# DoumanAsh/compu

Hardware: AMD Instinct MI355X
Metric: decompressed GB/s (whole node), batched 64 KiB DEFLATE blocks; % HBM peak (higher is better)
Workload: dtype u8

## Files before the change

compu_amd/csrc/api.hip:

```cpp
#include <stdio.h>
#include <stdlib.h>
#include <string.h>

#include <mutex>
#include <new>
#include <thread>
#include <vector>

#include "chip_internal.h"
#include "lz4_enc_core.h"

using namespace chip;

namespace {

struct Hooks {
    chip_malloc_fn malloc_fn = nullptr;
    chip_free_fn free_fn = nullptr;
    void *opaque = nullptr;
    void *alloc(size_t n) const { return malloc_fn ? malloc_fn(opaque, n) : malloc(n); }
    void release(void *p) const
    {
        if (!p) return;
        if (free_fn) free_fn(opaque, p);
        else free(p);
    }
};
std::mutex g_hooks_mu;
Hooks g_hooks;
Hooks current_hooks()
{
    std::lock_guard<std::mutex> lk(g_hooks_mu);
    return g_hooks;
}

bool device_ok()
{
    int n = 0;
    return hipGetDeviceCount(&n) == hipSuccess && n > 0;
}

struct Meta {
    uint64_t in_off, out_off;
    uint32_t in_len, out_cap, out_len, in_used;
    int32_t status;
    uint32_t resume[RESUME_WORDS];
};

BatchArgs batch_args(int format, size_t n, const void *in_base, const uint64_t *in_off, const uint32_t *in_len, void *out_base,
                     const uint64_t *out_off, const uint32_t *out_cap, uint32_t *out_len, uint32_t *in_used, int32_t *status)
{
    BatchArgs a;
    a.in_base = (const uint8_t *)in_base;
    a.in_off = in_off;
    a.in_len = in_len;
    a.out_base = (uint8_t *)out_base;
    a.out_off = out_off;
    a.out_cap = out_cap;
    a.out_len = out_len;
    a.in_used = in_used;
    a.status = status;
    a.n = (uint32_t)n;
    a.format = format;
    a.stats = nullptr;
    a.resume = nullptr;
#ifdef CHIP_STATS
    a.stats = getenv("CHIP_STATS_PTR") ? (unsigned long long *)strtoull(getenv("CHIP_STATS_PTR"), nullptr, 0) : nullptr;
#endif
    return a;
}

void pipes_trim();

}

extern "C" {

int chip_device_count(void)
{
    int n = 0;
    if (hipGetDeviceCount(&n) != hipSuccess) return 0;
    return n;
}

int chip_set_device(int device) { return hipSetDevice(device) == hipSuccess ? CHIP_OK : CHIP_E_NO_DEVICE; }

const char *chip_version(void) { return "compu-hip 0.1 (gfx950)"; }

void chip_set_allocator(chip_malloc_fn malloc_fn, chip_free_fn free_fn, void *opaque)
{
    std::lock_guard<std::mutex> lk(g_hooks_mu);
    g_hooks.malloc_fn = (malloc_fn && free_fn) ? malloc_fn : nullptr;
    g_hooks.free_fn = (malloc_fn && free_fn) ? free_fn : nullptr;
    g_hooks.opaque = (malloc_fn && free_fn) ? opaque : nullptr;
}

void *chip_device_alloc(size_t size)
{
    void *p = nullptr;
    if (hipMalloc(&p, size ? size : 4) != hipSuccess) return nullptr;
    return p;
}
void chip_device_free(void *ptr)
{
    if (ptr) (void)hipFree(ptr);
}
void *chip_pinned_alloc(size_t size)
{
    void *p = nullptr;
    if (hipHostMalloc(&p, size ? size : 4, hipHostMallocDefault) != hipSuccess) return nullptr;
    return p;
}
void chip_pinned_free(void *ptr)
{
    if (ptr) (void)hipHostFree(ptr);
}
int chip_memcpy_h2d(void *dst, const void *src, size_t size, void *stream)
{
    return hipMemcpyAsync(dst, src, size, hipMemcpyHostToDevice, (hipStream_t)stream) == hipSuccess ? CHIP_OK : CHIP_E_LAUNCH;
}
int chip_memcpy_d2h(void *dst, const void *src, size_t size, void *stream)
{
    return hipMemcpyAsync(dst, src, size, hipMemcpyDeviceToHost, (hipStream_t)stream) == hipSuccess ? CHIP_OK : CHIP_E_LAUNCH;
}
int chip_stream_sync(void *stream) { return hipStreamSynchronize((hipStream_t)stream) == hipSuccess ? CHIP_OK : CHIP_E_LAUNCH; }
int chip_trim(void)
{
    pipes_trim();
    return chip::release_scratch() == hipSuccess ? CHIP_OK : CHIP_E_LAUNCH;
}


int chip_decode_batch(int format, size_t n, const void *in_base, const uint64_t *in_off, const uint32_t *in_len,
                      void *out_base, const uint64_t *out_off, const uint32_t *out_cap, uint32_t *out_len,
                      uint32_t *in_used, int32_t *status, void *stream)
{
    return chip_decode_batch_ex(format, 0, n, in_base, in_off, in_len, out_base, out_off, out_cap, out_len, in_used, status, stream);
}

static bool members_flag_ok(int format, uint32_t flags)
{
    if ((format == CHIP_FMT_LZ4_BLOCK || format == CHIP_FMT_LZ4) && flags) return false;
    if (!(flags & CHIP_F_MEMBERS)) return true;
    if (flags & CHIP_F_COMPU_STATUS) return false;
    return format == CHIP_FMT_GZIP || format == CHIP_FMT_AUTO || format == CHIP_FMT_ZSTD || format == CHIP_FMT_DETECT;
}

int chip_decode_batch_ex(int format, uint32_t flags, size_t n, const void *in_base, const uint64_t *in_off, const uint32_t *in_len,
                         void *out_base, const uint64_t *out_off, const uint32_t *out_cap, uint32_t *out_len,
                         uint32_t *in_used, int32_t *status, void *stream)
{
    if (flags & ~(uint32_t)(CHIP_F_COMPU_STATUS | CHIP_F_MEMBERS)) return CHIP_E_INVALID;
    if (!members_flag_ok(format, flags)) return CHIP_E_INVALID;
    if (n == 0) return CHIP_OK;
    if (n > 0x7fffffffull || !in_base || !in_off || !in_len || !out_base || !out_off || !out_cap || !out_len || !in_used ||
        !status || ((uintptr_t)in_base & 3u))
        return CHIP_E_INVALID;
    if (!device_ok()) return CHIP_E_NO_DEVICE;
    BatchArgs a = batch_args(format, n, in_base, in_off, in_len, out_base, out_off, out_cap, out_len, in_used, status);
    a.flags = flags;
    hipError_t e;
    switch (format) {
    case CHIP_FMT_DEFLATE:
    case CHIP_FMT_ZLIB:
    case CHIP_FMT_GZIP:
    case CHIP_FMT_AUTO: e = launch_inflate(a, nullptr, (hipStream_t)stream); break;
    case CHIP_FMT_ZSTD: e = launch_zstd(a, nullptr, 0, (hipStream_t)stream); break;
    case CHIP_FMT_BROTLI: e = launch_brotli_decode(a, (hipStream_t)stream); break;
    case CHIP_FMT_LZ4_BLOCK:
    case CHIP_FMT_LZ4: e = launch_lz4(a, nullptr, (hipStream_t)stream); break;
    case CHIP_FMT_DETECT:
        e = launch_routed(a, nullptr, (hipStream_t)stream);
        break;
    default: return CHIP_E_INVALID;
    }
    return e == hipSuccess ? CHIP_OK : CHIP_E_LAUNCH;
}

int chip_decode_batch_sizes(int format, uint32_t flags, size_t n, const void *in_base, const uint64_t *in_off, const uint32_t *in_len,
                            uint64_t *out_size, uint32_t *in_used, int32_t *status, void *stream)
{
    if (flags & ~(uint32_t)CHIP_F_MEMBERS) return CHIP_E_INVALID;
    if (!members_flag_ok(format, flags)) return CHIP_E_INVALID;
    switch (format) {
    case CHIP_FMT_DEFLATE:
    case CHIP_FMT_ZLIB:
    case CHIP_FMT_GZIP:
    case CHIP_FMT_AUTO:
    case CHIP_FMT_ZSTD:
    case CHIP_FMT_LZ4_BLOCK:
    case CHIP_FMT_LZ4:
    case CHIP_FMT_DETECT: break;
    default: return CHIP_E_INVALID;
    }
    if (n == 0) return CHIP_OK;
    if (n > 0x7fffffffull || !in_base || !in_off || !in_len || !out_size || !in_used || !status || ((uintptr_t)in_base & 3u))
        return CHIP_E_INVALID;
    if (!device_ok()) return CHIP_E_NO_DEVICE;
    BatchArgs a = batch_args(format, n, in_base, in_off, in_len, nullptr, nullptr, nullptr, nullptr, in_used, status);
    a.flags = flags;
    hipError_t e;
    if (format == CHIP_FMT_ZSTD) e = launch_zstd(a, out_size, 0, (hipStream_t)stream);
    else if (format == CHIP_FMT_LZ4_BLOCK || format == CHIP_FMT_LZ4) e = launch_lz4(a, out_size, (hipStream_t)stream);
    else if (format == CHIP_FMT_DETECT) e = launch_routed(a, out_size, (hipStream_t)stream);
    else e = launch_inflate(a, out_size, (hipStream_t)stream);
    return e == hipSuccess ? CHIP_OK : CHIP_E_LAUNCH;
}

}

namespace {

struct DeviceGuard {
    int prev = -1;
    bool ok = true;
    explicit DeviceGuard(int device)
    {
        if (hipGetDevice(&prev) != hipSuccess) prev = -1;
        if (device >= 0 && device != prev) ok = hipSetDevice(device) == hipSuccess;
    }
// ... 1228 lines not shown
```

compu_amd/csrc/chip_internal.h:

```cpp
#pragma once
#include <hip/hip_runtime.h>
#include <stddef.h>
#include <stdint.h>

#include "../../include/compu_hip.h"
#include "zstd_enc_core.h"

namespace chip {

constexpr int32_t ST_RUNNING = 0x7fffffff;

constexpr int32_t Z_NEED_DICT = 2;
constexpr int32_t Z_DATA_ERROR = -3;

constexpr int32_t ZSTD_E_GENERIC = 1;
constexpr int32_t ZSTD_E_PREFIX_UNKNOWN = 10;
constexpr int32_t ZSTD_E_FRAMEPARAM_UNSUPPORTED = 14;
constexpr int32_t ZSTD_E_WINDOW_TOO_LARGE = 16;
constexpr int32_t ZSTD_E_CORRUPTION = 20;
constexpr int32_t ZSTD_E_CHECKSUM_WRONG = 22;
constexpr int32_t ZSTD_E_DICT_WRONG = 32;

constexpr uint32_t RESUME_WORDS = 6;

constexpr uint32_t ZRES_HDR = 24;
constexpr uint32_t ZSAVE_WORDS = 2312;
constexpr size_t ZRES_BYTES = (size_t)(ZRES_HDR + ZSAVE_WORDS) * 4 + 64;

struct BatchArgs {
    const uint8_t *in_base;
    const uint64_t *in_off;
    const uint32_t *in_len;
    uint8_t *out_base;
    const uint64_t *out_off;
    const uint32_t *out_cap;
    uint32_t *out_len;
    uint32_t *in_used;
    int32_t *status;
    uint32_t n;
    int32_t format;
    unsigned long long *stats;
    uint32_t *resume;
    const uint32_t *sel = nullptr;
    const uint32_t *sel_n = nullptr;
    uint32_t flags = 0;
};
struct ZTokArgs {
    const chip_zstd_block *blocks;
    const uint32_t *seq_base;
    uint32_t *tok;
    uint32_t *res;
    uint64_t window;
};
constexpr uint32_t ZTOK_SLOT_SLACK = 8736;
hipError_t launch_zstd_tokens(const BatchArgs &a, const ZTokArgs &tk, hipStream_t stream);
hipError_t launch_zstd_xxh(const uint8_t *p, uint32_t n, uint32_t *got, hipStream_t stream);
hipError_t launch_zstd_xxh_update(const uint8_t *p, uint32_t n, const chip_xxh64_state &st, chip_xxh64_state *out, hipStream_t stream);
constexpr uint32_t F_COMPU_STATUS = 1u;
constexpr uint32_t F_MEMBERS = 2u;

hipError_t launch_inflate(const BatchArgs &a, uint64_t *out_size, hipStream_t stream);
hipError_t enqueue_inflate_sizes(const BatchArgs &a, uint64_t *out_size, uint32_t *scratch, uint32_t *counter, uint32_t blocks, hipStream_t stream);
hipError_t enqueue_inflate_members(const BatchArgs &a, uint64_t *out_size, uint32_t *scratch, uint32_t *counter, uint32_t blocks, hipStream_t stream);
hipError_t enqueue_inflate_markers(const BatchArgs &a, const uint32_t *bit0, uint32_t *scratch, uint32_t *counter, uint32_t blocks, hipStream_t stream);
hipError_t launch_zstd(const BatchArgs &a, uint64_t *out_size, int window_log_max, hipStream_t stream);
hipError_t enqueue_zstd_sizes(const BatchArgs &a, uint64_t *out_size, int wlog_max, hipStream_t stream);
hipError_t enqueue_zstd_members(const BatchArgs &a, int wlog_max, hipStream_t stream);
hipError_t enqueue_zstd_members_sizes(const BatchArgs &a, uint64_t *out_size, int wlog_max, hipStream_t stream);
hipError_t launch_lz4(const BatchArgs &a, uint64_t *out_size, hipStream_t stream);
hipError_t launch_lz4_xxh(const uint8_t *p, uint64_t n, uint32_t *got, hipStream_t stream);
bool lz4_encode_args_ok(int format, int level, int strategy);
hipError_t launch_lz4_encode(const BatchArgs &a, int level, int strategy, hipStream_t stream);
hipError_t release_scratch();
void release_scratch_of(hipStream_t stream);
hipError_t launch_route(const BatchArgs &a, uint64_t *out_size, uint32_t *sel_inflate, uint32_t *sel_zstd, uint32_t *counts, hipStream_t stream);
hipError_t launch_routed(const BatchArgs &a, uint64_t *out_size, hipStream_t stream);
hipError_t launch_detect(size_t n, const uint8_t *in_base, const uint64_t *in_off, const uint32_t *in_len, int32_t *kind,
                         hipStream_t stream);
hipError_t launch_deflate_l1(const BatchArgs &a, int level, uint32_t flags, uint32_t check_seed, uint64_t total_before,
                             uint32_t *check_out, hipStream_t stream);

constexpr uint32_t ZF_FIRST = 1u, ZF_LAST = 2u, ZF_ONESHOT = 4u;
struct ZEncStream {
    uint32_t rep[3], pad;
    zenc::Xxh xxh;
};
hipError_t launch_zstd_encode(const BatchArgs &a, int level, int strategy, uint32_t wlog_single, uint32_t wlog_window, uint32_t flags,
                              ZEncStream *stream_state, hipStream_t stream);

struct BEncStream {
    uint32_t ring[4];
};
hipError_t launch_brotli_encode(const BatchArgs &a, int quality, int lgwin, uint32_t flags, BEncStream *stream_state, hipStream_t stream);

constexpr uint32_t BRES_WORDS = 16;
static_assert(BRES_WORDS <= ZRES_HDR, "the brotli checkpoint fits the header the streaming code copies");
hipError_t launch_brotli_decode(const BatchArgs &a, hipStream_t stream);
size_t brotli_scratch_bytes_of(hipStream_t stream);

__device__ __forceinline__ int32_t detect_kind(const uint8_t *b, uint32_t len)
{
    if (len < 2) return CHIP_DETECT_NONE;
    const uint32_t b0 = b[0], b1 = b[1];
    if (b0 == 0x1f && b1 == 0x8b) return CHIP_DETECT_GZIP;
    if (((b0 << 8) | b1) % 31 == 0 && (b0 & 0x8f) == 0x08 && b0 != 0x68) {
        const uint32_t rows[8] = {0x1d5b99d7u, 0x195795d3u, 0x155391cfu, 0x114f8dcbu, 0x0d4b89c7u, 0x094785c3u, 0x054381deu, 0x015e9cdau};
        const uint32_t r = rows[b0 >> 4];
        if (b1 == (r >> 24) || b1 == ((r >> 16) & 0xff) || b1 == ((r >> 8) & 0xff) || b1 == (r & 0xff)) return CHIP_DETECT_ZLIB;
    }
    if (len < 4) return CHIP_DETECT_NONE;
    return (b0 == 0x28 && b1 == 0xb5 && b[2] == 0x2f && b[3] == 0xfd) ? CHIP_DETECT_ZSTD : CHIP_DETECT_UNKNOWN;
}

#define LDS_AS __attribute__((address_space(3)))
#define GAS __attribute__((address_space(1)))

__device__ __forceinline__ uint32_t lane_id() { return threadIdx.x & 63u; }
__device__ __forceinline__ uint64_t lanemask_lt() { return (1ull << lane_id()) - 1ull; }
__device__ __forceinline__ uint32_t rdlane(uint32_t v, uint32_t l)
{
    return (uint32_t)__builtin_amdgcn_readlane((int)v, (int)l);
}
__device__ __forceinline__ uint32_t rdfirst(uint32_t v) { return (uint32_t)__builtin_amdgcn_readfirstlane((int)v); }
template <typename T>
__device__ __forceinline__ T *rdfirst_ptr(T *p)
{
    const uint64_t v = (uint64_t)(uintptr_t)p;
    return (T *)(uintptr_t)(((uint64_t)rdfirst((uint32_t)(v >> 32)) << 32) | rdfirst((uint32_t)v));
}

template <int CTRL, int ROW_MASK = 0xf>
__device__ __forceinline__ uint32_t dpp_or_zero(uint32_t v)
{
    return (uint32_t)__builtin_amdgcn_update_dpp(0, (int)v, CTRL, ROW_MASK, 0xf, false);
}

__device__ __forceinline__ uint32_t wave_incl_scan(uint32_t v)
{
    v += dpp_or_zero<0x111>(v);
    v += dpp_or_zero<0x112>(v);
    v += dpp_or_zero<0x114>(v);
    v += dpp_or_zero<0x118>(v);
    v += dpp_or_zero<0x142, 0xa>(v);
    v += dpp_or_zero<0x143, 0xc>(v);
    return v;
}

__device__ __forceinline__ uint32_t wave_incl_max_scan(uint32_t v)
{
    uint32_t t;
    t = dpp_or_zero<0x111>(v); v = v > t ? v : t;
    t = dpp_or_zero<0x112>(v); v = v > t ? v : t;
    t = dpp_or_zero<0x114>(v); v = v > t ? v : t;
    t = dpp_or_zero<0x118>(v); v = v > t ? v : t;
    t = dpp_or_zero<0x142, 0xa>(v); v = v > t ? v : t;
    t = dpp_or_zero<0x143, 0xc>(v); v = v > t ? v : t;
    return v;
}

__device__ __forceinline__ uint32_t wave_shr1(uint32_t v) { return dpp_or_zero<0x138>(v); }

#define WSYNC() __syncthreads()
#define LSYNC() asm volatile("s_waitcnt lgkmcnt(0)" ::: "memory")

}
```

compu_amd/csrc/inflate_unit.h:

```cpp
#pragma once
#include "chip_internal.h"
#include "wave_checksums.h"

namespace chip {

typedef uint32_t u32x2 __attribute__((ext_vector_type(2)));
typedef uint32_t u32x4 __attribute__((ext_vector_type(4)));
typedef u32x4 u32x4_u __attribute__((aligned(1)));
typedef u32x4 u32x4_a4 __attribute__((aligned(4)));
template <typename T>
__device__ __forceinline__ GAS T *rdfirst_gptr(T *p)
{
    return (GAS T *)rdfirst_ptr(p);
}

#ifndef CHIP_PHASE_FN
#define CHIP_PHASE_FN __attribute__((always_inline))
#endif

#ifndef CHIP_INFLATE_SPEC
#define CHIP_INFLATE_SPEC 0
#endif
#ifndef CHIP_INFLATE_MARKERS
#define CHIP_INFLATE_MARKERS 0
#endif
#if CHIP_INFLATE_SPEC
#define SPEC_PARAM , uint32_t &sp_reach
#define SPEC_ARG , sp_reach
#else
#define SPEC_PARAM
#define SPEC_ARG
#endif

#ifdef CHIP_STATS
#define STAT_DECL unsigned long long st_[24] = {0}; unsigned long long st_t0_ = 0
#define STAT_T0() (st_t0_ = __builtin_readcyclecounter())
#define STAT_ACC(i) do { unsigned long long n_ = __builtin_readcyclecounter(); st_[i] += n_ - st_t0_; st_t0_ = n_; } while (0)
#define STAT_ADD(i, v) (st_[i] += (unsigned long long)(v))
#define STAT_PARAM , unsigned long long *st_, unsigned long long &st_t0_
#define STAT_ARG , st_, st_t0_
#else
#define STAT_DECL
#define STAT_T0()
#define STAT_ACC(i)
#define STAT_ADD(i, v)
#define STAT_PARAM
#define STAT_ARG
#endif

enum : uint32_t { K_LIT = 0, K_LEN = 1, K_EOB = 2, K_BAD = 3 };
__device__ __forceinline__ constexpr uint32_t mk_entry(uint32_t cl, uint32_t eb, uint32_t kind, uint32_t base)
{
    return cl | (eb << 4) | (kind << 8) | (base << 16);
}

constexpr int LIT_ROOT = 9;
constexpr int DIST_ROOT = 8;
constexpr int CL_ROOT = 7;

constexpr uint32_t F_HALT = 1u << 15, F_INV = 1u << 26, F_LEN = 1u << 31;
constexpr uint32_t D_BAD = 1u << 10, D_LONG = 1u << 15;
static_assert(15 - LIT_ROOT < 8 && 15 - DIST_ROOT < 8, "a root entry's index bit count leaves its bits [4:3] clear");
static_assert((2u << (15 - DIST_ROOT)) - 2u < 256u, "the distance sub-tables fit the 256 units that a root entry's offset spans");

__device__ __forceinline__ uint32_t make_final(uint32_t sym, uint32_t len)
{
    if (sym < 256) return len | (len << 10) | (sym << 16);
    if (sym == 256) return len | (len << 10) | F_HALT;
    if (sym >= 286) return len | (len << 10) | F_HALT | F_INV;
    const uint32_t s = sym - 257;
    uint32_t eb = 0, base = 3 + s;
    if (s == 28) base = 258;
    else if (s >= 8) {
        eb = (s >> 2) - 1;
        base = 3 + ((4 + (s & 3)) << eb);
    }
    return len | (eb << 5) | ((len + eb) << 10) | ((512u | base) << 16) | F_LEN;
}
__device__ __forceinline__ uint32_t make_dist16(uint32_t sym, uint32_t len)
{
    if (sym >= 30) return len | D_BAD;
    if (sym < 4) return len | (sym << 8);
    return len | (((sym >> 1) - 1) << 4) | ((2 + (sym & 1)) << 8);
}

#ifndef CHIP_S_BITS
#define CHIP_S_BITS 320
#define CHIP_XT_BITS 1536
#define CHIP_XT_BITS_FIXED 3072
#define CHIP_ROW_TOKENS 256
#endif
constexpr uint32_t S_BITS = CHIP_S_BITS;
constexpr uint32_t XT_BITS = CHIP_XT_BITS;
#ifndef CHIP_XT_BITS_FIXED
#define CHIP_XT_BITS_FIXED CHIP_XT_BITS
#endif
constexpr uint32_t XT_BITS_FIXED = CHIP_XT_BITS_FIXED;
constexpr uint32_t ROW_TOKENS = CHIP_ROW_TOKENS;
static_assert(S_BITS % 32 == 0 && ROW_TOKENS % 4 == 0 && 64 * ROW_TOKENS < 65536, "geometry");
constexpr uint32_t SEG_WORDS = S_BITS / 32 + 1;
constexpr uint32_t SEG_SHIFT = 24;
constexpr uint32_t SEG_MAGIC = ((1u << SEG_SHIFT) + S_BITS - 1) / S_BITS;
constexpr bool seg_magic_ok()
{
    for (uint32_t x = 0; x < 64u * S_BITS + 4096u; x++)
        if (((x * SEG_MAGIC) >> SEG_SHIFT) != x / S_BITS) return false;
    return true;
}
static_assert(seg_magic_ok() && (64u * S_BITS + 4096u) * (uint64_t)SEG_MAGIC < (1ull << 32), "segment index by multiplication");
constexpr uint32_t WIN_DW = (31 + 64 * S_BITS + 48 + 96 + 31) / 32 + 3;
constexpr uint32_t HDR_IN_DW = 192;

constexpr size_t ROWS_WORDS = (size_t)64 * ROW_TOKENS;
static_assert(64ull * ROW_TOKENS * 258 < (1ull << 32), "count_tokens() sums a super-round's output lengths in 32 bits");
__device__ __forceinline__ uint32_t row_base(uint32_t l) { return (l >> 3) * (8u * ROW_TOKENS) + (l & 7u) * 4u; }
__device__ __forceinline__ uint32_t row_word(uint32_t k) { return k + (k >> 2) * 28u; }

__device__ __forceinline__ uint32_t tok_olen(uint32_t t) { return (t & 512u) ? t & 0x1ffu : 1u + (t >> 31); }

struct HuffMeta {
    uint32_t limit15[16];
    uint32_t offs[16];
    uint32_t maxlen;
};

#ifndef CHIP_CHUNK_BYTES
#define CHIP_CHUNK_BYTES 2560
#endif
#ifndef CHIP_COPY_LANE_MAX
#define CHIP_COPY_LANE_MAX 32
#endif
constexpr uint32_t CHUNK_BYTES = CHIP_CHUNK_BYTES;
constexpr uint32_t COPY_LANE_MAX = CHIP_COPY_LANE_MAX;
constexpr uint32_t MQ_CAP = 128;
constexpr uint32_t IMG_WORDS = CHUNK_BYTES / 4 + 8;
constexpr uint32_t TOK_RING = 4;
static_assert(CHUNK_BYTES % 4 == 0 && CHUNK_BYTES >= 1024 && COPY_LANE_MAX % 16 == 0 && IMG_WORDS % 2 == 0, "geometry");

constexpr uint32_t FLUSH_BYTES = 4 * (IMG_WORDS + 2 * MQ_CAP + 64 * TOK_RING + 128 + 4);
constexpr uint32_t HDR_BYTES = 4 * HDR_IN_DW + 4 * (1 << CL_ROOT) + 80 + sizeof(HuffMeta) + 64 + 320 + 2 * 288 + 2 * 32 + 2 * sizeof(HuffMeta);
constexpr uint32_t PHASE_BYTES = 8 * WIN_DW > FLUSH_BYTES ? (8 * WIN_DW > HDR_BYTES ? 8 * WIN_DW : HDR_BYTES) : (FLUSH_BYTES > HDR_BYTES ? FLUSH_BYTES : HDR_BYTES);
#ifndef CHIP_LDS_BYTES
#define CHIP_LDS_BYTES 8960
#endif
constexpr uint32_t POOL_WORDS = (CHIP_LDS_BYTES - 2 * 512 - 2 * 256 - PHASE_BYTES) / 4;
constexpr uint32_t POOL_U16 = 2 * POOL_WORDS;
constexpr uint32_t DIST_SUB_BYTES = 2 * (POOL_U16 - 256);

struct alignas(16) WaveLds {
    union {
        struct {
            uint32_t win[WIN_DW];
            uint32_t bm[WIN_DW];
        } w;
        struct {
            uint32_t inbuf[HDR_IN_DW];
            uint32_t cl_lut[1 << CL_ROOT];
            uint32_t cl_sorted[20];
            HuffMeta cl_h;
            uint32_t count[16];
            uint8_t lens[320];
            uint16_t lit_sorted[288];
            uint16_t dist_sorted[32];
            HuffMeta lit_h, dist_h;
        } hdr;
        struct {
            uint32_t out[IMG_WORDS];
            uint2 mq[MQ_CAP];
            uint32_t tok[64 * TOK_RING];
            uint32_t pk[128];
            uint32_t trash[4];
        } fl;
        uint32_t phase_words_[PHASE_BYTES / 4];
    };
    uint16_t lit_root[1 << LIT_ROOT];
    uint16_t dist_root[1 << DIST_ROOT];
    uint32_t pool[POOL_WORDS];
};
static_assert(sizeof(WaveLds) <= CHIP_LDS_BYTES, "the waves per CU that CHIP_LDS_BYTES stands for");
static_assert(POOL_WORDS >= 413 + 142, "the tables of any valid block fit");
#ifndef CHIP_EXP_ALLOW_SMALL_LDS
static_assert(sizeof(WaveLds) >= 2048 * 4, "wave_crc32 needs 8 KB");
#endif

__device__ __forceinline__ uint32_t canon_index(const HuffMeta &H, uint32_t x15, uint32_t &l)
{
    l = 1;
    if (x15 >= H.limit15[15]) return 0xffffffffu;
#pragma unroll
    for (int j = 1; j < 15; j++) l += (x15 >= H.limit15[j]) ? 1u : 0u;
    return H.offs[l] + ((x15 - H.limit15[l - 1]) >> (15 - l));
}

struct CanonLim {
    uint32_t lim[16];
};
__device__ __forceinline__ CanonLim canon_limits(const HuffMeta &H)
{
    CanonLim c;
#pragma unroll
    for (int j = 0; j < 16; j++) c.lim[j] = rdfirst(H.limit15[j]);
    return c;
}
template <int LO, int HI>
__device__ __forceinline__ uint32_t canon_index_in(const HuffMeta &H, const CanonLim &c, uint32_t x15, uint32_t &l)
{
    l = LO;
#pragma unroll
    for (int j = LO; j < HI; j++) l += (x15 >= c.lim[j]) ? 1u : 0u;
    return H.offs[l] + ((x15 - H.limit15[l - 1]) >> (15 - l));
}

template <typename SortedT, typename MakeT>
__device__ __forceinline__ int canon_prep(uint32_t *count, const uint8_t *lens, int n_, bool code_lengths, SortedT *sorted, HuffMeta &H, MakeT make STAT_PARAM)
{
    const uint32_t lane = lane_id();
    const int n = (int)rdfirst((uint32_t)n_);
    if (lane < 16) count[lane] = 0;
    WSYNC();
    for (int s = lane; s < n; s += 64) {
        uint32_t l = lens[s];
        if (l) atomicAdd(&count[l], 1u);
    }
    WSYNC();
    const uint32_t c = lane >= 1 && lane <= 15 ? count[lane] : 0u;
    const uint32_t cincl = wave_incl_scan(c);
    const uint32_t off = cincl - c;
    const uint32_t lim = wave_incl_scan(lane <= 15 ? c << (15u - (lane & 15u)) : 0u);
    const uint32_t present = (uint32_t)__ballot(c != 0);
    const uint32_t maxlen = present ? 31u - (uint32_t)__clz((int)present) : 0u;
    const bool over = __any(lane <= 15 && lim > 32768u);
    const int left = rdlane(lim, 15) < 32768u ? 1 : 0;
    if (lane <= 15) {
        H.limit15[lane] = lim;
        H.offs[lane] = off;
        count[lane] = off;
    }
    if (lane == 0) H.maxlen = maxlen;
    WSYNC();
    if (maxlen == 0) return 1;
    if (over) return -1;
    if (left > 0 && (code_lengths || maxlen != 1)) return -1;
    for (int base = 0; base < n; base += 64) {
        STAT_ADD(19, 1);
        const int s = base + (int)lane;
        const uint32_t l = s < n ? lens[s] : 0;
        uint64_t same = ~0ull;
#pragma unroll
        for (uint32_t b = 0; b < 4; b++) {
            const bool bit = (l >> b) & 1u;
            const uint64_t m = __ballot(bit);
// ... 698 lines not shown
                nfirst = before < npieces ? nx : 0xffffffffu;
            }
            asm volatile("s_waitcnt vmcnt(0)" ::: "memory");
            slot_r = 0;
#pragma unroll
            for (uint32_t k = 0; k < TOK_RING; k++) fetch(k);
        }
        const uint32_t xcap = cap - (opos - mis);
        {
            const uint32_t xe = run < xcap ? run : xcap;
            for (uint32_t xq = 16u + 16u * lane; xq + 16u <= xe; xq += 1024u) *(GAS u32x4_a4 *)(base + xq) = *(const LDS_AS u32x4 *)(img + xq);
            const uint32_t xt = xe < 16u ? 16u : xe & ~15u;
            const uint32_t xb = lane < 16u ? lane : xt + (lane - 16u);
            if (lane < 32u && xb >= mis && xb < xe) ((GAS uint8_t *)base)[xb] = img[xb];
        }
        WSYNC();
        STAT_ACC(18);
        opos += run - mis;
        opos_ = opos;
        const bool no_room = opos > cap || (too_far && opos == cap);
        if (no_room || too_far) {
            if (no_room) {
                opos_ = cap;
                ovf[0] = cstart;
                ovf[1] = mis;
                ovf[2] = xcap;
            }
            status = no_room ? CHIP_NEED_OUTPUT : Z_DATA_ERROR;
            return false;
        }
        if (c0 >= ntok) return true;
    }
}
constexpr size_t SCRATCH_WORDS = ROWS_WORDS;


enum : uint32_t { R_JOIN = 1, R_LIMIT = 2, R_EOB = 3, R_NEED_INPUT = 4, R_BAD = 5 };

__device__ CHIP_PHASE_FN uint32_t walk_round(WaveLds &L, const InWin &w, const uint32_t B_, const uint32_t end_bit_, uint32_t *rows_, const uint32_t xt_bits,
                                             uint32_t &ntok_out, uint32_t &term_why, uint32_t &term_pos STAT_PARAM)
{
    const uint32_t lane = lane_id();
    const uint32_t B = rdfirst(B_), end_bit = rdfirst(end_bit_);
    GAS const uint32_t *const g32 = rdfirst_gptr(w.g32);
    const uint32_t total_dw = rdfirst(w.total_dw);
    GAS uint32_t *const myrow = rdfirst_gptr(rows_) + row_base(lane);
    const uint32_t D0 = B >> 5;
    WSYNC();
    {
        constexpr uint32_t WIN_Q = WIN_DW / 4, WIN_R = WIN_DW % 4;
        constexpr uint32_t BM_A = (WIN_DW + 3u) & ~3u;
        constexpr uint32_t BM_Q = (2u * WIN_DW - BM_A) / 4, BM_TAIL = (2u * WIN_DW - BM_A) % 4;
        constexpr uint32_t EDGE_LO = WIN_R + (BM_A - WIN_DW);
        constexpr uint32_t EDGE_LANES = 4u + EDGE_LO + BM_TAIL;
        constexpr uint32_t PER_LANE = (WIN_Q + 63) / 64;
        static_assert(offsetof(WaveLds, w.win) == 0 && offsetof(WaveLds, w.bm) == 4 * WIN_DW && BM_Q <= WIN_Q && EDGE_LANES <= 64, "window staging");
        uint32_t *const ww = L.w.win;
        const uint32_t rem = total_dw - D0;
        static_assert(PER_LANE <= 4, "the quads per lane below");
        auto quad = [&](uint32_t j) -> u32x4 {
            const uint32_t k = 64u * j + lane;
            if ((64u * j + 63u < WIN_Q || k < WIN_Q) && 4u * k + 4u <= rem) return *(GAS const u32x4_a4 *)(g32 + D0 + 4u * k);
            return u32x4{0, 0, 0, 0};
        };
        const u32x4 v0 = quad(0), v1 = quad(1), v2 = quad(2), v3 = quad(3);
        uint32_t ni = 4u * (rem >> 2) + lane;
        bool nput = ni < rem && ni < 4u * WIN_Q;
        if (lane >= 4u) {
            const uint32_t j = lane - 4u;
            ni = j < EDGE_LO ? 4u * WIN_Q + j : 2u * WIN_DW - BM_TAIL + (j - EDGE_LO);
            nput = j < EDGE_LO + BM_TAIL;
        }
        uint32_t nv = 0;
        if (nput && ni < rem && ni < WIN_DW) nv = g32[D0 + ni];
#pragma unroll
        for (uint32_t j = 0; j < PER_LANE; j++) {
            const uint32_t k = 64u * j + lane;
            if (64u * j + 63u < WIN_Q || k < WIN_Q) *(u32x4 *)(ww + 4u * k) = j == 0 ? v0 : j == 1 ? v1 : j == 2 ? v2 : v3;
            if (64u * j + 63u < BM_Q || k < BM_Q) *(u32x4 *)(ww + BM_A + 4u * k) = u32x4{0, 0, 0, 0};
        }
        if (nput) ww[ni] = nv;
    }
    LSYNC();
    STAT_ACC(1);
    STAT_ADD(8, 1);
    const uint32_t s0 = B + lane * S_BITS;
    const uint32_t own_end = s0 + S_BITS;
    uint32_t hard = own_end + xt_bits;
    {
        const uint32_t sr_end = B + 64u * S_BITS;
        hard = hard < sr_end ? hard : sr_end;
        hard = hard < end_bit ? hard : end_bit;
    }
    const uint32_t wbase = 32u * D0;
    const uint32_t own_end_r = own_end - wbase, hard_r = hard - wbase;
    uint32_t q = s0 - wbase, tl = 0, nst = 0;
    uint32_t jb = 0, z = 0;
    bool run = s0 < end_bit;
    uint32_t nx;
    {
        const uint32_t *wp = (const uint32_t *)((const uint8_t *)L.w.win + ((q >> 3) & ~3u));
        nx = __builtin_amdgcn_alignbit(wp[1], wp[0], q);
    }
    auto token = [&](uint32_t &tok) -> bool {
        const uint32_t p = q;
        const uint32_t a = (p >> 3) & ~3u;
        const uint32_t bit = 1u << (p & 31u);
        const uint32_t mine = p < own_end_r ? bit : 0u;
        const uint32_t old = atomicOr((uint32_t *)((uint8_t *)L.w.bm + a), mine);
        jb = old & bit & ~mine;
        const uint32_t *wp = (const uint32_t *)((const uint8_t *)L.w.win + a);
        const uint32_t d0 = wp[0], d1 = wp[1], d2 = wp[2];
        const uint32_t lo = __builtin_amdgcn_alignbit(d1, d0, p), hi = __builtin_amdgcn_alignbit(d2, d1, p);
        const uint32_t r = L.lit_root[nx & ((1u << LIT_ROOT) - 1u)];
        const uint32_t e = pool_at(L, r, nx);
        const uint32_t n1 = __builtin_amdgcn_ubfe(e, 10, 5);
        const uint32_t msk = (uint32_t)((int32_t)e >> 31);
        const uint32_t w2 = __builtin_amdgcn_alignbit(hi, lo, n1);
        uint32_t m = L.dist_root[w2 & ((1u << DIST_ROOT) - 1u)] & msk;
#ifndef CHIP_EXP_NO_PAIR
        const uint32_t p2 = p + n1;
        const uint32_t r2 = L.lit_root[w2 & ((1u << LIT_ROOT) - 1u)];
        const uint32_t mw2 = *(const uint32_t *)((const uint8_t *)L.w.bm + ((p2 >> 3) & ~3u));
#endif
        if (__any((m & D_LONG) != 0)) {
            asm volatile("; long distance codes");
            if (m & D_LONG) m = dist_sub_at(L, m, w2);
        }
#ifndef CHIP_EXP_NO_PAIR
        const uint32_t e2 = pool_at(L, r2, w2);
        const uint32_t mk2 = __builtin_amdgcn_ubfe(mw2, p2, 1);
#endif
        const uint32_t cl2 = m & 15u, eb2 = __builtin_amdgcn_ubfe(m, 4, 4);
        const uint32_t dm1 = ((m >> 8) << eb2) + __builtin_amdgcn_ubfe(w2, cl2, eb2);
        z = (e & (F_HALT | F_INV)) | (m & D_BAD);
        tl = n1 + cl2 + eb2;
#ifndef CHIP_EXP_NO_PAIR
        const uint32_t n2 = __builtin_amdgcn_ubfe(e2, 10, 5);
        const bool pair = ((e | e2) & (F_LEN | F_HALT)) == 0 && p2 + n2 <= hard_r && mk2 == 0;
        tl += pair ? n2 : 0u;
        const uint32_t pr = pair ? (e2 & 0x00ff0000u) | 0x80000000u : 0u;
#else
        const uint32_t pr = 0;
#endif
        static_assert((15 + 5) + (15 + 13) == 48 && 64 - 48 >= LIT_ROOT + (15 - LIT_ROOT), "the next step's index bits are in hi:lo");
        nx = (uint32_t)((((uint64_t)hi << 32) | lo) >> (tl & 63u));
        q = p + tl;
        if ((jb | z) != 0 || q > hard_r) return false;
        const uint32_t v = __builtin_amdgcn_ubfe(lo, e, e >> 5) + __builtin_amdgcn_ubfe(e, 16, 10);
        tok = (dm1 << 10) | v | pr;
        return true;
    };
    bool full = false;
    while (__any(run)) {
        STAT_ADD(11, 1);
        uint32_t t4[4];
#pragma unroll
        for (int k = 0; k < 4; k++) asm volatile("" : "=v"(t4[k]));
        uint32_t took = 0;
        if (run) {
            if (nst + 4u > ROW_TOKENS) {
                run = false;
                full = true;
            } else {
                bool ok = token(t4[0]);
                if (ok) {
                    took = 1;
                    ok = token(t4[1]);
                    if (ok) {
                        took = 2;
                        ok = token(t4[2]);
                        if (ok) {
                            took = 3;
                            ok = token(t4[3]);
                            if (ok) took = 4;
                        }
                    }
                }
                run = ok;
            }
        }
        if (took) *(GAS u32x4 *)(myrow + 8u * nst) = u32x4{t4[0], t4[1], t4[2], t4[3]};
        nst += took;
    }
    const bool dropped = s0 < end_bit && !full;
    const uint32_t pn = q + wbase;
    const uint32_t p = pn - (dropped ? tl : 0u);
    uint32_t why = R_LIMIT;
    if (s0 < end_bit && !full) {
        if (jb) why = R_JOIN;
        else if (pn > end_bit) why = R_NEED_INPUT;
        else if (z) why = z == F_HALT ? (uint32_t)R_EOB : (uint32_t)R_BAD;
    }
    STAT_ADD(21, __popcll(__ballot(nst != 0)));
    STAT_ACC(2);
    const uint32_t rel = p - B;
    const uint32_t jl = why == R_JOIN ? (__umul24(rel, SEG_MAGIC) >> SEG_SHIFT) & 63u : lane;
    uint32_t a_join = 0;
    if (__any(why == R_JOIN)) {
        const uint32_t sj = B + jl * S_BITS;
        const uint32_t w0 = (sj >> 5) - D0;
        const uint32_t lo_cut = sj & 31u;
        const uint32_t nb = p - (sj & ~31u);
#pragma unroll
        for (uint32_t t = 0; t < SEG_WORDS; t++) {
            uint32_t mw = L.w.bm[w0 + t];
            if (t == 0) mw &= ~0u << lo_cut;
            const int32_t k = (int32_t)nb - 32 * (int32_t)t;
            const uint32_t keep = k <= 0 ? 0u : k >= 32 ? 0xffffffffu : (1u << k) - 1u;
            a_join += __popc(mw & keep);
        }
        if (why != R_JOIN) a_join = 0;
    }
    uint32_t node = 0;
    {
        uint32_t pw = jl;
#pragma unroll
        for (int r = 0; r < 6; r++) {
            const uint32_t nx = lane_gather(pw, node);
            if ((lane >> r) & 1u) node = nx;
            pw = lane_gather(pw, pw);
        }
    }
    const uint32_t prev = wave_shr1(node);
    const bool fresh = lane == 0 || node != prev;
    const uint32_t e_nst = lane_gather(nst, node);
    const uint32_t g_a0 = lane_gather(a_join, prev);
    const uint32_t e_a0 = lane == 0 ? 0u : g_a0;
    const uint32_t cnt = (fresh && e_nst > e_a0) ? e_nst - e_a0 : 0u;
    const uint32_t incl = wave_incl_scan(cnt);
    const uint64_t nonempty = __ballot(cnt != 0);
    WSYNC();
    if (cnt) {
        const uint32_t k = (uint32_t)__popcll(nonempty & lanemask_lt()), first = incl - cnt;
        L.fl.pk[2u * k] = first;
        L.fl.pk[2u * k + 1u] = ((e_a0 - first) & 0xffffu) | (row_base(node) << 16);
    }
    const uint32_t kz = rdlane(node, 63);
    term_why = rdlane(why, kz);
    term_pos = rdlane(p, kz);
    ntok_out = rdlane(incl, 63u);
    WSYNC();
    STAT_ACC(3);
    STAT_ADD(9, __popcll(nonempty));
    STAT_ADD(10, ntok_out);
    return (uint32_t)__popcll(nonempty);
}

__device__ CHIP_PHASE_FN bool count_tokens(WaveLds &L, const uint32_t *grow_, uint32_t ntok_, uint32_t npieces_, uint64_t &osize, int32_t &status SPEC_PARAM)
{
    const uint32_t lane = lane_id();
    GAS const uint32_t *const grow = rdfirst_gptr(grow_);
    const uint32_t ntok = rdfirst(ntok_), npieces = rdfirst(npieces_);
    if (ntok == 0) return true;
    const bool have = lane < npieces;
    const uint32_t pfirst = have ? L.fl.pk[2u * lane] : ntok;
    const uint32_t pdelta = have ? L.fl.pk[2u * lane + 1u] : 0u;
    const uint32_t pnext = lane + 1u < npieces ? L.fl.pk[2u * lane + 2u] : ntok;
    const uint32_t k0 = (pfirst + pdelta) & 0xffffu;
    const uint32_t kend = k0 + (have ? pnext - pfirst : 0u);
    GAS const uint32_t *const row = grow + (pdelta >> 16);
    uint32_t sum = 0;
    for (uint32_t kq = k0 & ~3u; __any(kq < kend); kq += 4u) {
        if (kq < kend) {
            const u32x4 t = *(GAS const u32x4 *)(row + 8u * kq);
            const uint32_t t4[4] = {t.x, t.y, t.z, t.w};
#pragma unroll
            for (uint32_t j = 0; j < 4; j++)
                if (kq + j >= k0 && kq + j < kend) sum += tok_olen(t4[j]);
        }
    }
    const uint32_t incl = wave_incl_scan(sum);
    const uint32_t olo = rdfirst((uint32_t)osize), ohi = rdfirst((uint32_t)(osize >> 32));
#if CHIP_INFLATE_SPEC
    if (ohi == 0 && olo < 32768u) {
        uint32_t at = olo + incl - sum, reach = 0;
        for (uint32_t kq = k0 & ~3u; __any(kq < kend); kq += 4u) {
            if (kq < kend) {
                const u32x4 t = *(GAS const u32x4 *)(row + 8u * kq);
                const uint32_t t4[4] = {t.x, t.y, t.z, t.w};
#pragma unroll
                for (uint32_t j = 0; j < 4; j++)
                    if (kq + j >= k0 && kq + j < kend) {
                        const uint32_t dist = __builtin_amdgcn_ubfe(t4[j], 10, 16) + 1u;
                        if ((t4[j] & 512u) != 0 && dist > at && dist - at > reach) reach = dist - at;
                        at += tok_olen(t4[j]);
                    }
            }
        }
        const uint32_t far = rdlane(wave_incl_max_scan(reach), 63u);
        if (far > sp_reach) sp_reach = far;
    }
    (void)status;
#else
    if (ohi == 0 && olo < 32768u) {
        uint32_t at = olo + incl - sum, badat = 0xffffffffu;
        for (uint32_t kq = k0 & ~3u; __any(kq < kend); kq += 4u) {
            if (kq < kend) {
                const u32x4 t = *(GAS const u32x4 *)(row + 8u * kq);
                const uint32_t t4[4] = {t.x, t.y, t.z, t.w};
#pragma unroll
                for (uint32_t j = 0; j < 4; j++)
                    if (kq + j >= k0 && kq + j < kend) {
                        const bool ismatch = (t4[j] & 512u) != 0;
                        if (ismatch && __builtin_amdgcn_ubfe(t4[j], 10, 16) + 1u > at && badat == 0xffffffffu) badat = at;
                        at += tok_olen(t4[j]);
                    }
            }
        }
        const uint64_t badm = __ballot(badat != 0xffffffffu);
        if (badm) {
            osize = rdlane(badat, (uint32_t)__ffsll((long long)badm) - 1u);
            status = Z_DATA_ERROR;
            return false;
        }
    }
#endif
    osize = (((uint64_t)ohi << 32) | olo) + rdlane(incl, 63u);
    return true;
}

#if CHIP_INFLATE_MARKERS
#define MSYNC() __builtin_amdgcn_fence(__ATOMIC_SEQ_CST, "workgroup")
constexpr uint32_t MARK = 0x8000u, MARK_WINDOW = 32768u;
constexpr uint32_t LANE_COPY16 = 32;

__device__ __forceinline__ void copy_match16(GAS uint16_t *gout, uint32_t x, uint32_t len, uint32_t dist)
{
    const uint32_t lane = lane_id();
    const int32_t sx = (int32_t)x - (int32_t)dist;
    for (uint32_t i = lane; i < len; i += 64) {
        const int32_t s = sx + (int32_t)(dist >= len ? i : small_mod(i, dist));
        const uint16_t v = s < 0 ? (uint16_t)(MARK | (uint32_t)(s + (int32_t)MARK_WINDOW)) : gout[s];
        gout[x + i] = v;
    }
    MSYNC();
}
// ... 408 lines not shown
            win_ensure(L, w, pos, 316 * 14 + 160);
            static_assert(offsetof(WaveLds, hdr.lens) % 4 == 0 && sizeof(L.hdr.lens) == 320, "lens[] is zeroed a dword at a time");
            for (uint32_t k = lane; k < 320 / 4; k += 64) ((uint32_t *)L.hdr.lens)[k] = 0;
            WSYNC();
            while (have < total) {
                STAT_ADD(7, 1);
                const uint32_t bp = pos + lane;
                uint32_t lo, hi;
                win_bits(L, w, bp, lo, hi);
                const uint32_t e = L.hdr.cl_lut[lo & 127u];
                const uint32_t cl = e & 15u, sym = e >> 16;
                const uint32_t eb = sym < 16 ? 0u : sym == 16 ? 2u : sym == 17 ? 3u : 7u;
                const uint32_t tl = cl + eb;
                const uint32_t run = sym < 16 ? 1u : (sym == 18 ? 11u : 3u) + bfe(lo, cl, eb);
                const uint32_t nx = lane + tl;
                uint32_t nth = 0;
                {
                    uint32_t pw = nx < 64u ? nx : 64u;
#pragma unroll
                    for (int r = 0; r < 6; r++) {
                        const uint32_t g1 = lane_gather(pw, nth & 63u), g2 = lane_gather(pw, pw & 63u);
                        if ((lane >> r) & 1u) nth = nth < 64u ? g1 : 64u;
                        pw = pw < 64u ? g2 : 64u;
                    }
                }
                uint8_t *const onflag = (uint8_t *)L.hdr.count;
                if (lane < 16) L.hdr.count[lane] = 0;
                LSYNC();
                if (nth < 64u) onflag[nth] = 1;
                LSYNC();
                const bool on = onflag[lane] != 0;
                const uint32_t c = on ? run : 0u;
                const uint32_t incl = wave_incl_scan(c);
                const uint32_t start = have + incl - c;
                const bool need = on && start < total;
                uint32_t bad = 0;
                if (need && bp + tl > end_bit) bad = 1;
                else if (need && sym == 16 && start == 0) bad = 2;
                else if (need && sym >= 16 && start + run > total) bad = 2;
                const uint64_t badm = __ballot(bad != 0);
                const uint32_t fb = badm ? (uint32_t)__ffsll((long long)badm) - 1u : 64u;
                const bool ok = need && lane < fb;
                const uint32_t expl = sym < 16 ? sym : 0u;
                const uint32_t m = wave_incl_max_scan((ok && sym != 16) ? (((lane + 1u) << 8) | expl) : 0u);
                const uint32_t v = sym == 16 ? (m ? m & 0xffu : prevlen) : expl;
                if (ok && sym < 16) L.hdr.lens[start] = (uint8_t)sym;
                if (ok && sym == 16)
                    for (uint32_t j = 0; j < run; j++) L.hdr.lens[start + j] = (uint8_t)v;
                if (badm) {
                    status = rdlane(bad, fb) == 1 ? (int32_t)CHIP_NEED_INPUT : Z_DATA_ERROR;
                    break;
                }
                const uint64_t okm = __ballot(ok);
                const uint32_t lv = 63u - (uint32_t)__clzll((long long)okm);
                have = rdlane(start + run, lv);
                pos += lv + rdlane(tl, lv);
                prevlen = rdlane(v, lv);
            }
            if (status != ST_RUNNING) break;
            WSYNC();
            STAT_ACC(4);
            if (rdfirst(L.hdr.lens[256]) == 0) {
                status = Z_DATA_ERROR;
                break;
            }
        }
        if (build) {
            eob_len = rdfirst(L.hdr.lens[256]);
            uint32_t used = 0;
            const int r1 = build_litlen(L, L.hdr.lens, (int)nlen, used STAT_ARG);
            const int r2 = r1 ? r1 : build_dist(L, L.hdr.lens + nlen, (int)ndist, used STAT_ARG);
            if (r1 || r2) {
                status = Z_DATA_ERROR;
                break;
            }
            STAT_ACC(5);
        }
        STAT_ACC(0);
        __builtin_amdgcn_s_setprio(0);
        decode_block<SIZES>(L, w, pos, end_bit, gout, opos, cap, status, scratch, tables == 1 ? XT_BITS_FIXED : XT_BITS, eob_len, a.flags, osize STAT_ARG SPEC_ARG);
        __builtin_amdgcn_s_setprio(2);
        STAT_T0();
    }
    __builtin_amdgcn_s_setprio(0);
    STAT_ACC(0);
    if (SIZES && status == CHIP_FINISHED && wrap) {
        uint32_t k = (pos - start_bit + 7u) >> 3;
        if (wrap == 1) {
            if (in_len - k < 4) status = CHIP_NEED_INPUT;
            k += 4;
        } else {
            if (in_len - k < 8) status = CHIP_NEED_INPUT;
            else {
                uint32_t isize = gin[k + 4] | ((uint32_t)gin[k + 5] << 8) | ((uint32_t)gin[k + 6] << 16) | ((uint32_t)gin[k + 7] << 24);
                if (rdfirst(isize) != (uint32_t)osize) status = Z_DATA_ERROR;
            }
            k += 8;
        }
        pos = start_bit + k * 8u;
    }
    if (!SIZES && status == CHIP_FINISHED && wrap) {
        uint32_t k = (pos - start_bit + 7u) >> 3;
        uint32_t need = wrap == 2 ? 8u : 4u;
        if (in_len - k < need && wrap == 1) {
            status = CHIP_NEED_INPUT;
        } else if (wrap == 1) {
            uint32_t want = ((uint32_t)gin[k] << 24) | ((uint32_t)gin[k + 1] << 16) | ((uint32_t)gin[k + 2] << 8) | gin[k + 3];
            const uint32_t c0 = run_cov - out_dropped;
            if (rdfirst(wave_adler32(gout + c0, opos - c0, resumed ? run_check : 1u)) != rdfirst(want)) status = Z_DATA_ERROR;
            k += 4;
        } else if (in_len - k < 4) {
            status = CHIP_NEED_INPUT;
        } else {
            uint32_t want = gin[k] | ((uint32_t)gin[k + 1] << 8) | ((uint32_t)gin[k + 2] << 16) | ((uint32_t)gin[k + 3] << 24);
            const uint32_t c0 = run_cov - out_dropped;
            if (rdfirst(wave_crc32((LDS_AS uint32_t *)&L, gout + c0, opos - c0, resumed ? run_check : 0u)) != rdfirst(want)) status = Z_DATA_ERROR;
            else if (in_len - k < 8) status = CHIP_NEED_INPUT;
            else {
                uint32_t isize = gin[k + 4] | ((uint32_t)gin[k + 5] << 8) | ((uint32_t)gin[k + 6] << 16) | ((uint32_t)gin[k + 7] << 24);
                if (rdfirst(isize) != out_dropped + opos) status = Z_DATA_ERROR;
            }
            k += 8;
        }
        pos = start_bit + k * 8u;
    }
#if CHIP_INFLATE_MEMBERS
    if (status == CHIP_FINISHED && wrap == 2) {
        const uint32_t k = (pos - start_bit) >> 3;
        if (in_len - k >= 2 && rdfirst(gin[k]) == 0x1fu && rdfirst(gin[k + 1]) == 0x8bu) {
            WSYNC();
            if constexpr (SIZES) {
                osize_members += osize;
                osize = 0;
            } else {
                gout += opos;
                cap -= opos;
                opos_members += opos;
                opos = 0;
            }
            format = CHIP_FMT_GZIP;
            status = ST_RUNNING;
            last = false;
            tables = 0;
            w.win0 = 0xffffffffu;
            goto next_member;
        }
    }
    opos += opos_members;
    osize += osize_members;
#endif
    STAT_ACC(6);
#ifdef CHIP_STATS
    if (a.stats && lane == 0)
        for (int k = 0; k < 24; k++) a.stats[(size_t)u * 24 + k] = st_[k];
#endif
    if (!SIZES && a.resume) {
        const bool cont = status == CHIP_NEED_INPUT || status == CHIP_NEED_OUTPUT;
        uint32_t *rs = a.resume + RESUME_WORDS * u;
        if (!resumed) run_check = wrap == 1 ? 1u : 0u;
        const uint32_t c0 = run_cov - out_dropped;
        if (cont && wrap && ck_bit != 0 && ck_opos > c0) {
            run_check = wrap == 1 ? wave_adler32(gout + c0, ck_opos - c0, run_check) : wave_crc32((LDS_AS uint32_t *)&L, gout + c0, ck_opos - c0, run_check);
            run_cov = out_dropped + ck_opos;
        }
        if (lane == 0) {
            rs[0] = cont ? ck_bit : 0u;
            rs[1] = cont ? ck_opos : 0u;
            rs[2] = wrap;
            rs[3] = run_check;
            rs[4] = run_cov;
            rs[5] = out_dropped;
        }
    }
    uint32_t used = (pos - start_bit + 7u) >> 3;
    if (used > in_len) used = in_len;
    if (!SIZES && (a.flags & F_COMPU_STATUS)) {
        if (status == CHIP_NEED_OUTPUT && used == in_len) status = CHIP_NEED_INPUT;
        else if (status == CHIP_NEED_INPUT && in_len == 0) status = CHIP_NEED_OUTPUT;
    }
#if CHIP_INFLATE_INDEX
    if (lane == 0) {
        ix.walk[0] = ix_n;
        ix.walk[1] = status == CHIP_FINISHED ? ix_end : 0u;
        ix.walk[2] = wrap;
    }
#endif
#if CHIP_INFLATE_SPEC
    if (lane == 0)
        sp.out[u] = SpecOut{osize, sp_bit0 + (status == CHIP_FINISHED ? sp_end : ck_bit), sp_kind, sp_link, status, sp_reach, wrap, sp_first};
#endif
    if (lane == 0) {
        if constexpr (SIZES) out_size[u] = osize;
        else a.out_len[u] = opos;
        a.in_used[u] = status == CHIP_NEED_INPUT ? in_len : used;
        a.status[u] = status;
    }
}

}
```

Before: 375.6.

## Decode remaining few token chains wave-cooperatively with speculative per-bit-offset decode

Result: no change. 379.3, median of 6 (+1.0%).

```diff
diff --git a/compu_amd/csrc/api.hip b/compu_amd/csrc/api.hip
--- a/compu_amd/csrc/api.hip
+++ b/compu_amd/csrc/api.hip
@@ -66,6 +66,7 @@
     a.resume = nullptr;
 #ifdef CHIP_STATS
     a.stats = getenv("CHIP_STATS_PTR") ? (unsigned long long *)strtoull(getenv("CHIP_STATS_PTR"), nullptr, 0) : nullptr;
+    if (getenv("CHIP_STATS_SLOTS") && atoi(getenv("CHIP_STATS_SLOTS")) == 26) a.stats_slots = 26;
 #endif
     return a;
 }
diff --git a/compu_amd/csrc/chip_internal.h b/compu_amd/csrc/chip_internal.h
--- a/compu_amd/csrc/chip_internal.h
+++ b/compu_amd/csrc/chip_internal.h
@@ -40,6 +40,7 @@
     uint32_t n;
     int32_t format;
     unsigned long long *stats;
+    uint32_t stats_slots = 24;
     uint32_t *resume;
     const uint32_t *sel = nullptr;
     const uint32_t *sel_n = nullptr;
diff --git a/compu_amd/csrc/inflate_unit.h b/compu_amd/csrc/inflate_unit.h
--- a/compu_amd/csrc/inflate_unit.h
+++ b/compu_amd/csrc/inflate_unit.h
@@ -33,7 +33,7 @@
 #endif
 
 #ifdef CHIP_STATS
-#define STAT_DECL unsigned long long st_[24] = {0}; unsigned long long st_t0_ = 0
+#define STAT_DECL unsigned long long st_[26] = {0}; unsigned long long st_t0_ = 0
 #define STAT_T0() (st_t0_ = __builtin_readcyclecounter())
 #define STAT_ACC(i) do { unsigned long long n_ = __builtin_readcyclecounter(); st_[i] += n_ - st_t0_; st_t0_ = n_; } while (0)
 #define STAT_ADD(i, v) (st_[i] += (unsigned long long)(v))
@@ -97,6 +97,11 @@
 #endif
 constexpr uint32_t XT_BITS_FIXED = CHIP_XT_BITS_FIXED;
 constexpr uint32_t ROW_TOKENS = CHIP_ROW_TOKENS;
+#ifndef CHIP_DENSE_T
+#define CHIP_DENSE_T 2
+#endif
+static_assert(CHIP_DENSE_T >= 1 && CHIP_DENSE_T <= 64, "a number of chains");
+constexpr uint32_t DENSE_T = CHIP_DENSE_T;
 static_assert(S_BITS % 32 == 0 && ROW_TOKENS % 4 == 0 && 64 * ROW_TOKENS < 65536, "geometry");
 constexpr uint32_t SEG_WORDS = S_BITS / 32 + 1;
 constexpr uint32_t SEG_SHIFT = 24;
@@ -1101,7 +1106,9 @@
         return true;
     };
     bool full = false;
-    while (__any(run)) {
+    uint64_t runm = __ballot(run);
+    bool more = runm != 0;
+    while (more) {
         STAT_ADD(11, 1);
         uint32_t t4[4];
 #pragma unroll
@@ -1131,7 +1138,111 @@
         }
         if (took) *(GAS u32x4 *)(myrow + 8u * nst) = u32x4{t4[0], t4[1], t4[2], t4[3]};
         nst += took;
-    }
+        runm = __ballot(run);
+        more = runm != 0;
+#ifndef CHIP_EXP_NO_DENSE
+        if (more && (uint32_t)__popcll(runm) <= DENSE_T) {
+            asm volatile("; few chains");
+            more = __ballot(run && q < own_end_r) != 0;
+        }
+#endif
+    }
+#ifndef CHIP_EXP_NO_DENSE
+    if (runm != 0) {
+        static_assert((31u + 64u * S_BITS + 63u) / 32u + 2u < WIN_DW, "a dense step's window reads stay inside the window");
+        GAS uint32_t *const rows = rdfirst_gptr(rows_);
+        uint64_t todo = runm, fullm = 0;
+        do {
+            const uint32_t own = (uint32_t)__ffsll((long long)todo) - 1u;
+            todo &= todo - 1ull;
+            uint32_t cq = rdlane(q, own), cn = rdlane(nst, own);
+            const uint32_t chard = rdlane(hard_r, own);
+            GAS uint32_t *const crow = rows + row_base(own);
+            const bool mine = lane == own;
+            for (;;) {
+                STAT_ADD(24, 1);
+                const uint32_t p = cq + lane;
+                const uint32_t a = (p >> 3) & ~3u;
+                const uint32_t *wp = (const uint32_t *)((const uint8_t *)L.w.win + a);
+                const uint32_t mw = *(const uint32_t *)((const uint8_t *)L.w.bm + a);
+                const uint32_t d0 = wp[0], d1 = wp[1], d2 = wp[2];
+                const uint32_t lo = __builtin_amdgcn_alignbit(d1, d0, p), hi = __builtin_amdgcn_alignbit(d2, d1, p);
+                const uint32_t r = L.lit_root[lo & ((1u << LIT_ROOT) - 1u)];
+                const uint32_t e = pool_at(L, r, lo);
+                const uint32_t n1 = __builtin_amdgcn_ubfe(e, 10, 5);
+                const uint32_t msk = (uint32_t)((int32_t)e >> 31);
+                const uint32_t w2 = __builtin_amdgcn_alignbit(hi, lo, n1);
+                uint32_t m = L.dist_root[w2 & ((1u << DIST_ROOT) - 1u)] & msk;
+                if (__any((m & D_LONG) != 0)) {
+                    asm volatile("; long distance codes, dense");
+                    if (m & D_LONG) m = dist_sub_at(L, m, w2);
+                }
+                const uint32_t cl2 = m & 15u, eb2 = __builtin_amdgcn_ubfe(m, 4, 4);
+                const uint32_t dm1 = ((m >> 8) << eb2) + __builtin_amdgcn_ubfe(w2, cl2, eb2);
+                const uint32_t dtl = n1 + cl2 + eb2;
+                const uint32_t zz = __builtin_amdgcn_ubfe(mw, p, 1) | (e & (F_HALT | F_INV)) | (m & D_BAD);
+                const uint32_t dts = dtl | ((zz != 0 || p + dtl > chard) ? 64u : 0u);
+                const uint32_t tok = (dm1 << 10) | (__builtin_amdgcn_ubfe(lo, e, e >> 5) + __builtin_amdgcn_ubfe(e, 16, 10));
+                enum : uint32_t { GOES_ON = 0, ROW_FULL = 1, STOPPED = 2 };
+                const uint32_t room = ROW_TOKENS - cn;
+                uint64_t taken = 0;
+                uint32_t s = 0, x = 0, ends = GOES_ON;
+                if (room >= 64u) {
+                    uint32_t at;
+                    do {
+                        at = s;
+                        x = rdlane(dts, s);
+                        taken |= 1ull << s;
+                        s += x;
+                    } while (s < 64u);
+                    if (x & 64u) {
+                        ends = STOPPED;
+                        s = at;
+                        taken ^= 1ull << at;
+                    }
+                } else {
+                    for (uint32_t left = room; s < 64u; left--) {
+                        if (left == 0) {
+                            ends = ROW_FULL;
+                            break;
+                        }
+                        x = rdlane(dts, s);
+                        if (x & 64u) {
+                            ends = STOPPED;
+                            break;
+                        }
+                        taken |= 1ull << s;
+                        s += x;
+                    }
+                }
+                const uint32_t cnt = (uint32_t)__popcll(taken);
+                if (__builtin_amdgcn_inverse_ballot_w64(taken)) {
+                    const uint32_t k = cn + __builtin_amdgcn_mbcnt_hi((uint32_t)(taken >> 32), __builtin_amdgcn_mbcnt_lo((uint32_t)taken, 0u));
+                    crow[row_word(k)] = tok;
+                }
+                STAT_ADD(25, cnt);
+                cn += cnt;
+                if (ends != GOES_ON) {
+                    if (ends == STOPPED) {
+                        const uint32_t tls = x & 63u, zs = rdlane(zz, s);
+                        q = mine ? cq + s + tls : q;
+                        tl = mine ? tls : tl;
+                        jb = mine ? zs & 1u : jb;
+                        z = mine ? zs & ~1u : z;
+                    } else {
+                        q = mine ? cq + s : q;
+                        fullm |= 1ull << own;
+                    }
+                    nst = mine ? cn : nst;
+                    break;
+                }
+                cq += s;
+            }
+        } while (todo != 0);
+        run = false;
+        full = full || ((fullm >> lane) & 1ull) != 0;
+    }
+#endif
     const bool dropped = s0 < end_bit && !full;
     const uint32_t pn = q + wbase;
     const uint32_t p = pn - (dropped ? tl : 0u);
@@ -1846,7 +1957,7 @@
     STAT_ACC(6);
 #ifdef CHIP_STATS
     if (a.stats && lane == 0)
-        for (int k = 0; k < 24; k++) a.stats[(size_t)u * 24 + k] = st_[k];
+        for (uint32_t k = 0; k < a.stats_slots; k++) a.stats[(size_t)u * a.stats_slots + k] = st_[k];
 #endif
     if (!SIZES && a.resume) {
         const bool cont = status == CHIP_NEED_INPUT || status == CHIP_NEED_OUTPUT;
```
